# WilliamFlinchbaugh/Deep-RL-Battlespace

Hardware: AMD Instinct MI355X
Metric: agent-steps/sec (higher is better)
Workload: dtype f64/i16

## Files before the change

deep-rl-battlespace_amd/build.py:

```python
import os
import subprocess
import sys

HERE = os.path.dirname(os.path.abspath(__file__))
CSRC = os.path.join(HERE, "csrc")
INCLUDE = os.path.join(os.path.dirname(HERE), "include")
LIB = os.path.join(CSRC, "libbattlespace_hip.so")
COMMON = ["-O3", "--offload-arch=gfx950", "-fPIC", "-std=c++17", "-Wall", "-Wno-unused-function"]
STEP_FLAGS = ["-ffp-contract=off", "-mllvm", "-disable-machine-licm", "-mllvm", "-amdgpu-mfma-vgpr-form", "-mllvm", "-amdgpu-kernarg-preload-count=15"]
PER_CALL_FLAGS = STEP_FLAGS + ["-mllvm", "-amdgpu-sched-strategy=max-ilp"]
SOURCES = [(os.path.join(CSRC, "bsx_kernels.hip"), STEP_FLAGS),
           (os.path.join(CSRC, "bsx_step_per_call.hip"), PER_CALL_FLAGS),
           (os.path.join(CSRC, "bsx_step_multi_tick.hip"), STEP_FLAGS),
           (os.path.join(CSRC, "bsx_step_two_wave.hip"), PER_CALL_FLAGS),
           (os.path.join(CSRC, "bsx_step_rollout.hip"), STEP_FLAGS),
           (os.path.join(CSRC, "bsx_actor.hip"), ["-ffp-contract=off", "-mllvm", "-amdgpu-mfma-vgpr-form"]),
           (os.path.join(CSRC, "bsx_actor_grad.hip"), ["-ffp-contract=off", "-mllvm", "-amdgpu-mfma-vgpr-form"]),
           (os.path.join(CSRC, "bsx_replay.hip"), []),
           (os.path.join(CSRC, "bsx_advantage.hip"), ["-ffp-contract=off"]),
           (os.path.join(CSRC, "bsx_ppo_head.hip"), []),
           (os.path.join(CSRC, "bsx_adam_step.hip"), []),
           (os.path.join(CSRC, "bsx_ddpg_head.hip"), []),
           (os.path.join(CSRC, "bsx_shuffle.hip"), [])]


def _stale():
    if not os.path.exists(LIB):
        return True
    t = os.path.getmtime(LIB)
    import glob
    deps = [src for src, _ in SOURCES] + glob.glob(os.path.join(CSRC, "*.h")) + glob.glob(os.path.join(CSRC, "*.inl")) + \
        [os.path.join(INCLUDE, "battlespace_hip.h"), os.path.abspath(__file__)]
    return any(os.path.getmtime(d) > t for d in deps)


def build(force=False, verbose=False):
    if not force and not _stale():
        return LIB
    hipcc = os.environ.get("HIPCC", "/opt/rocm/bin/hipcc")
    from concurrent.futures import ThreadPoolExecutor

    def compile_one(item):
        src, extra = item
        obj = os.path.splitext(src)[0] + ".o"
        cmd = [hipcc, *COMMON, *extra, "-I", INCLUDE, "-c", src, "-o", obj]
        if verbose:
            print(" ".join(cmd), flush=True)
        subprocess.run(cmd, check=True)
        return obj
    with ThreadPoolExecutor(max_workers=len(SOURCES)) as pool:
        objs = list(pool.map(compile_one, SOURCES))
    cmd = [hipcc, "--offload-arch=gfx950", "-shared", "-fPIC", *objs, "-o", LIB]
    if verbose:
        print(" ".join(cmd), flush=True)
    subprocess.run(cmd, check=True)
    return LIB


if __name__ == "__main__":
    print(build(force="--force" in sys.argv, verbose=True))
```

deep-rl-battlespace_amd/csrc/bsx_kernels.hip:

```cpp

#include <array>
#include <mutex>
#include <unordered_map>

#include "bsx_config.h"
#include "bsx_args.h"
#include "bsx_state.h"
#include "bsx_rng.h"
#include "bsx_geometry.h"
#include "bsx_instinct.h"
#include "bsx_step_kernel.h"
#define BSX_INST_PER_CALL
#define BSX_INST_MULTI_TICK
#define BSX_INST_ROLLOUT
#include "bsx_step_split.h"
#define BSX_INST_SPLIT_MANY
#define BSX_INST_SPLIT
#define BSX_INST_SPLIT_CONT
#ifdef BSX_VARIANT
#define BSX_INST_KW
#else
#define BSX_INST_KW extern
#endif
#include "bsx_step_instances.h"
// ... 58 lines not shown
    if (!p.observe_only) {
        const int lane = tid & 63;
        const int64_t wb = int64_t(blockIdx.x) * (TPB / 64) + (tid >> 6);
        const unsigned long long resetting = __ballot(doit);
        if (resetting != 0ull && wb < wave_blocks(p.E, n)) {
            uint2* const pool = p.st.bent + size_t(wb) * POOL_CAP;
            const int pc = int(p.st.bcnt[wb]);
            int wpos = 0;
            for (int base = 0; base < pc; base += 64) {
                const int w = base + lane;
                const uint2 en = pool[w < pc ? w : 0];
                const bool stay = w < pc && ((resetting >> (en.x >> ENT_OWNER_SHIFT)) & 1ull) == 0ull;
                const unsigned long long kb = __ballot(stay);
                const int ps = wpos + __popcll(kb & ((1ull << lane) - 1ull));
                if (stay) pool[ps] = en;
                wpos += __popcll(kb);
            }
            if (lane == 0) p.st.bcnt[wb] = uint32_t(wpos);
        }
    }
    s_x[tid] = x; s_y[tid] = y; s_hp[tid] = valid ? hp : 0;
    __syncthreads();
    if (valid && p.obs) {
        const int team = a < n ? 0 : 1;
        write_obs<0>(p.obs + g * size_t(3 * n + 2), n, hp > 0, x, y, dir, a,
                     team == 0 ? er.bbx : er.brx, team == 0 ? er.bby : er.bry, gl, s_x, s_y, s_hp);
    }
}

__global__ void bsx_mark_done_kernel(uint2* envd, int64_t E) {
    const int64_t e = int64_t(blockIdx.x) * blockDim.x + threadIdx.x;
    if (e < E) envd[e] = make_uint2(1u << 27, 0u);
}

struct ExportArgs { StatePtrs st; int64_t E; int n; BsxExport out; int tie_tick; };

__global__ __launch_bounds__(TPB) void bsx_export_kernel(const ExportArgs p) {
    const int A = 2 * p.n;
    const size_t EA = size_t(p.E) * A;
    const size_t g = size_t(blockIdx.x) * TPB + threadIdx.x;
    if (g >= EA) return;
    const int64_t e = int64_t(g / A);
    const int a = int(g % A);
    const uint2 pw = p.st.plane[g];
    int x, y, hp;
    double dir;
    unpack_plane(pw, x, y, hp, dir);
    if (pw.y & PLANE_FRAC) dir = p.st.pdirf[g];
    const BsxExport& o = p.out;
    if (o.px) o.px[g] = x;
    if (o.py) o.py[g] = y;
    if (o.pdir) o.pdir[g] = dir;
    if (o.php) o.php[g] = hp;
    if (o.palive) o.palive[g] = hp > 0;
    const uint2 dw = p.st.envd[e];
    const EnvU ev = unpack_env(p.st.envc[e], dw.x);
    const int ptick = ev.tick - ((ev.done && ev.winner == BSX_WINNER_TIE && ev.tick >= p.tie_tick) ? 1 : 0);
    for (int k = 0; k < K; ++k) {
        const size_t i = g * K + k;
        if (o.bl_live) o.bl_live[i] = 0;
        if (o.bl_x) o.bl_x[i] = 0;
        if (o.bl_y) o.bl_y[i] = 0;
        if (o.bl_dir) o.bl_dir[i] = 0.0;
    }
    const int G = group_width(p.n), EPB = 64 / G;
    const int64_t wb = e / EPB;
    const uint32_t me = uint32_t(int(e % EPB) * G + a);
    const uint2* const pool = p.st.bent + size_t(wb) * POOL_CAP;
    const int cnt = int(p.st.bcnt[wb]);
    for (int j2 = 0; j2 < cnt; ++j2) {
        const uint32_t w = pool[j2].x;
        const int age = bullet_age(w);
        if ((w >> ENT_OWNER_SHIFT) != me || age == int(TOMBSTONE_AGE)) continue;
        int slot = (ptick - age + 1) % K;
        if (slot < 0) slot += K;
        const size_t i = g * K + slot;
        if (o.bl_live) o.bl_live[i] = 1;
        if (o.bl_x) o.bl_x[i] = bullet_x(w);
        if (o.bl_y) o.bl_y[i] = bullet_y(w);
        if (o.bl_dir) o.bl_dir[i] = p.st.bdir[size_t(slot) * EA + g];
    }
    if (a == 0) {
        if (o.base_xy) { o.base_xy[4 * e] = ev.brx; o.base_xy[4 * e + 1] = ev.bry; o.base_xy[4 * e + 2] = ev.bbx; o.base_xy[4 * e + 3] = ev.bby; }
        if (o.bhp) { o.bhp[2 * e] = ev.bhp_r; o.bhp[2 * e + 1] = ev.bhp_b; }
        if (o.tick) o.tick[e] = ev.tick;
        if (o.env_done) o.env_done[e] = ev.done;
        if (o.winner) o.winner[e] = ev.winner;
        if (o.counters) {
            const int* c4 = p.st.cnt + 4 * e;
            o.counters[4 * e] = c4[0]; o.counters[4 * e + 1] = c4[1]; o.counters[4 * e + 2] = c4[2]; o.counters[4 * e + 3] = c4[3];
        }
    }
}

struct InstinctArgs {
    const float* obs; void* actions; const double* rnd; int64_t E; int n; int team; int out_kind; int continuous;
    uint64_t seed; uint64_t seq; const uint64_t* seq_base; int64_t env_offset;
};

__global__ __launch_bounds__(TPB) void bsx_instinct_kernel(const InstinctArgs p) {
    const int A = 2 * p.n, D = 3 * p.n + 2;
    const size_t g = size_t(blockIdx.x) * TPB + threadIdx.x;
    if (g >= size_t(p.E) * A) return;
    const int a = int(g % A);
    const int tm = a < p.n ? 0 : 1;
    if (p.team != 2 && p.team != tm) return;
    const float* o = p.obs + g * D;
    double td, ta;
    const int act = instinct_choose([&](int k) { return o[k]; }, p.n, td, ta);
    if (!p.continuous) {
        if (p.out_kind == BSX_ACT_I32) static_cast<int32_t*>(p.actions)[g] = act;
        else static_cast<float4*>(p.actions)[g] = one_hot_scores(act);
        return;
    }
    double r0, n0, n1, n2;
    if (p.rnd) { r0 = p.rnd[4 * g]; n0 = p.rnd[4 * g + 1]; n1 = p.rnd[4 * g + 2]; n2 = p.rnd[4 * g + 3]; }
    else instinct_continuous_draws(p.seed, p.seq + (p.seq_base ? *p.seq_base : 0ull), uint64_t(p.env_offset) * uint64_t(A) + g, r0, n0, n1, n2);
    double* out = static_cast<double*>(p.actions) + 3 * g;
    instinct_continuous_action(td, ta, r0, n0, n1, n2, out[0], out[1], out[2]);
}

std::mutex g_family_mu;
std::unordered_map<const void*, int> g_family;
inline void family_forget(const void* state) {
    std::lock_guard<std::mutex> lk(g_family_mu);
    g_family.erase(state);
}
inline bool family_claim(const void* state, bool cont) {
    std::lock_guard<std::mutex> lk(g_family_mu);
    int& f = g_family[state];
    if (f == 0) f = cont ? 2 : 1;
    return f == (cont ? 2 : 1);
}
inline int grid_for(int64_t E, int n) {
    const int epb = TPB / group_width(n);
    return int((E + epb - 1) / epb);
}

inline bool narrow_offsets_ok(int64_t E, int n, uint32_t flags) {
    return !(flags & BSX_F_WIDE_OFFSETS) && uint64_t(E) * uint64_t(2 * n) * 200ull <= 0xFFFFFFFFull;
}
constexpr int64_t SPLIT_MAX_GAMES = 114688, SPLIT_MANY_MAX_GAMES = 65536, SPLIT_CONT_MAX_GAMES = 81920;
constexpr int64_t SPLIT_DRAW_MAX_GAMES = 98304;
constexpr int64_t SPLIT_MANY_FORM2_FROM = 32768;
template <bool CONT, bool MULTI>
inline bool split_applies(int n, const StepArgs& a, int64_t bound) {
    if (n != 1 || (a.flags & BSX_F_ONE_WAVE)) return false;
    if (CONT) return !MULTI && bound <= SPLIT_CONT_MAX_GAMES;
    return bound <= (MULTI ? SPLIT_MANY_MAX_GAMES : SPLIT_MAX_GAMES);
}

using StepKernel = void (*)(BSX_STEP_KERNEL_PARAMS);

template <class F>
StepKernel by_team_and_offsets(int n, bool off32, F f) {
    const auto w = [&](auto N) { return off32 ? f(N, std::true_type{}) : f(N, std::false_type{}); };
    switch (n) {
        case 1: return w(std::integral_constant<int, 1>{});
        case 2: return w(std::integral_constant<int, 2>{});
        case 3: return w(std::integral_constant<int, 3>{});
        case 4: return w(std::integral_constant<int, 4>{});
        default: return w(std::integral_constant<int, 0>{});
    }
}

template <bool CONT, bool MULTI, bool ACTOR, bool LG>
int launch_for_n(const StepArgs& a, int64_t bound, void* stream) {
    const int n = a.n;
    const bool two_wave = !ACTOR && split_applies<CONT, MULTI>(n, a, bound);
    const StepKernel k = by_team_and_offsets(n, narrow_offsets_ok(a.E, n, a.flags), [&](auto N_, auto OFF32_) -> StepKernel {
        constexpr int N = decltype(N_)::value;
        constexpr bool OFF32 = decltype(OFF32_)::value;
        if constexpr (ACTOR) {
            if constexpr (N == 0) return nullptr;
            else return bsx_step_kernel<N, CONT, true, true, false, OFF32>;
        } else {
            if constexpr (N == 1 && !(CONT && MULTI)) {
                if (two_wave) {
                    if constexpr (MULTI)
                        return bound > SPLIT_MANY_FORM2_FROM ? bsx_step_split_kernel<LG, OFF32, 2>
                                                             : bsx_step_split_kernel<LG, OFF32, 1>;
                    else if constexpr (CONT)
                        return bsx_step_split_kernel<false, OFF32, 0, true, true>;
                    else
                        return bound <= SPLIT_DRAW_MAX_GAMES ? bsx_step_split_kernel<LG, OFF32, 0, false, true>
                                                             : bsx_step_split_kernel<LG, OFF32, 0>;
                }
            }
            return bsx_step_kernel<N, CONT, MULTI, false, LG, OFF32>;
        }
    });
    const StepGeometry geo = step_geometry(ACTOR ? FORM_ROLLOUT : (two_wave ? FORM_TWO_WAVE : FORM_ONE_WAVE), bound, n);
    const dim3 grid(unsigned(geo.groups));
    const dim3 block(SPB * geo.waves);
    hipLaunchKernelGGL(k, grid, block, 0, static_cast<hipStream_t>(stream),
                       bound, a.st.envc, a.st.envd, a.st.plane, a.actions, a.st.bent, a.st.bcnt, a.action_kind, a);
    return int(hipGetLastError());
}

StepArgs step_args(void* state, int64_t E, int n, int T, float* rew, uint8_t* done, uint8_t* env_done, uint8_t* winner,
                   uint8_t* env_done_t, const BsxRewards* cfg, uint32_t flags, uint64_t seed, int64_t env_offset) {
    StepArgs a{};
    a.st = state_ptrs(state, E, n);
    a.E = E; a.n = n; a.T = T;
    a.rew = rew; a.done = done; a.env_done = env_done; a.winner = winner; a.env_done_t = env_done_t;
    a.cfg = *cfg; a.flags = flags; a.seed = seed; a.env_offset = env_offset; a.tie_tick = tie_tick_const(n);
    a.scripted_team = -1;
    return a;
}

struct StepCall { int64_t first = 0, count = -1; int T = 0; int store_all = 0; uint8_t* env_done_t = nullptr; };

template <bool CONT>
int step(const StepCall& c, void* state, int64_t E, int n, const void* actions, int action_kind, const double* u, float* obs, float* rew,
         uint8_t* done, uint8_t* env_done, uint8_t* winner, const BsxRewards* cfg, uint32_t flags, uint64_t seed, int64_t env_offset,
         void* stream) {
    const int T = c.T;
    const int64_t first = c.first, count = c.count < 0 ? E - first : c.count;
    if (T < 0 || T > BSX_MAX_T || first < 0 || count <= 0 || first > E - count || (first & 255) || ((first || count != E) && T != 0))
        return BSX_E_ARG;
    if (!obs || !rew || !done || !cfg || (!actions && (T || !(flags & BSX_F_EMPTY_CALL)))) return BSX_E_ARG;
    if (const int rc = check_games(state, E, n)) return rc;
    if (!aligned(obs, 4) || !aligned(rew, 4) || (u && !aligned(u, 8))) return BSX_E_ALIGN;
    if (!CONT && action_kind == BSX_ACT_LOGITS_F32 && !aligned(actions, 16)) return BSX_E_ALIGN;
    if (!CONT && action_kind != BSX_ACT_I32 && action_kind != BSX_ACT_LOGITS_F32) return BSX_E_ARG;
    if (CONT && action_kind != BSX_ACT_F32 && action_kind != BSX_ACT_F64 && action_kind != BSX_ACT_F32X4) return BSX_E_ARG;
    if (CONT && action_kind == BSX_ACT_F32X4 && !aligned(actions, 16)) return BSX_E_ALIGN;
    if (!family_claim(state, CONT)) return BSX_E_FAMILY;
    StepArgs a = step_args(state, E, n, T, rew, done, env_done, winner, c.env_done_t, cfg, flags, seed, env_offset);
    a.actions = actions; a.action_kind = action_kind; a.u = u; a.obs = obs;
    if (!actions) { a.actions = state; a.action_kind = -1; }
    const int64_t EA = E * 2 * n;
    a.act_tb = EA * (CONT ? (action_kind == BSX_ACT_F32 ? 12 : (action_kind == BSX_ACT_F64 ? 24 : 16)) : (action_kind == BSX_ACT_I32 ? 4 : 16));
    a.u_ts = EA;
    a.obs_ts = c.store_all ? EA * (3 * n + 2) : 0; a.rew_ts = c.store_all ? EA : 0; a.done_ts = c.store_all ? EA : 0;
    if (first) {
        const int64_t fa = first * 2 * n;
        const int64_t fb = first / (64 / group_width(n));
        a.st.envc += first; a.st.envd += first; a.st.cnt += 4 * first; a.st.plane += fa; a.st.pdirf += fa;
        a.st.bcnt += fb; a.st.bent += fb * POOL_CAP; a.st.bdir += fa; a.st.bd += fa;
        if (actions) a.actions = static_cast<const char*>(actions) + fa * (a.act_tb / EA);
        if (u) a.u += fa;
        a.obs += fa * (3 * n + 2); a.rew += fa; a.done += fa;
        if (env_done) a.env_done += first;
        if (winner) a.winner += first;
        a.env_offset += first;
    }
    const bool lg = !CONT && action_kind == BSX_ACT_LOGITS_F32;
    if (T == 0) return lg ? launch_for_n<CONT, false, false, !CONT>(a, count, stream) : launch_for_n<CONT, false, false, false>(a, count, stream);
    return lg ? launch_for_n<CONT, true, false, !CONT>(a, count, stream) : launch_for_n<CONT, true, false, false>(a, count, stream);
}

template <bool CONT>
int rollout(void* state, int64_t E, int n, int T, const float* weights, int precision, int scripted_team, uint64_t scripted_seed, float* obs,
            float* scores, float* rew, uint8_t* done, uint8_t* env_done, uint8_t* winner, uint8_t* env_done_t, const BsxRewards* cfg,
            uint32_t flags, const BsxActorNoise* noise, uint64_t actor_seed, uint64_t seq, const uint64_t* seq_base, uint64_t seed,
            int64_t env_offset, void* stream, bool gauss = false, const BsxGaussianHead* head = nullptr) {
    if (T < 1 || T > BSX_MAX_T || !weights || !obs || !scores || !rew || !done || !cfg || (flags & BSX_F_EMPTY_CALL) ||
        (precision != BSX_ACTOR_F32 && precision != BSX_ACTOR_BF16X3 && precision != BSX_ACTOR_BF16X6) || scripted_team < -1 || scripted_team > 1)
        return BSX_E_ARG;
    if (gauss && (!head || !head->log_std)) return BSX_E_ARG;
    if (const int rc = check_games(state, E, n, 256, ROLLOUT_MAX_N)) return rc;
    if (!aligned(weights, 16) || !aligned(scores, 16) || !aligned(obs, 4) || !aligned(rew, 4)) return BSX_E_ALIGN;
    BsxActorNoise nz = {};
    if (noise) nz = *noise;
    if (gauss) {
        if (nz.gaussian_std > 0.f || nz.ou_scale > 0.f || nz.sample_mode != 0 || nz.u_inject || nz.logp) return BSX_E_ARG;
        if (!aligned(head->log_std, 4) || (head->logp && !aligned(head->logp, 4))) return BSX_E_ALIGN;
    }
    if (nz.ou_scale > 0.f && (!nz.ou_state || !aligned(nz.ou_state, 16))) return nz.ou_state ? BSX_E_ALIGN : BSX_E_ARG;
    if (nz.z_inject || nz.u_inject) return BSX_E_ARG;
    if (nz.sample_mode != 0 && (nz.sample_mode != 1 || !(nz.temperature > 0.f) || CONT)) return BSX_E_ARG;
    if ((nz.logp && !aligned(nz.logp, 4)) || (nz.value_weights && !aligned(nz.value_weights, 16))) return BSX_E_ALIGN;
    if (nz.value_weights && (n != 1 || !nz.value || !aligned(nz.value, 4))) return BSX_E_ARG;
    if (!family_claim(state, CONT)) return BSX_E_FAMILY;
    const int64_t EA = E * 2 * n, D = 3 * n + 2;
    StepArgs a = step_args(state, E, n, T, rew, done, env_done, winner, env_done_t, cfg, flags, seed, env_offset);
    a.action_kind = CONT ? BSX_ACT_F32X4 : BSX_ACT_LOGITS_F32;
    a.obs = obs + EA * D; a.obs_ts = EA * D; a.rew_ts = EA; a.done_ts = EA;
    a.aw = weights; a.aprec = precision; a.scripted_team = scripted_team; a.obs0 = obs; a.scores = scores; a.scores_ts = EA * 4; a.nz = nz;
    a.aseed = actor_seed; a.aseq = seq; a.aseq_base = seq_base; a.iseed = scripted_seed;
    if (gauss) a.gh = *head;
    return launch_for_n<CONT, true, true, false>(a, E, stream);
}

const std::array<double2, 361>& heading_table() {
    static const std::array<double2, 361> lut = [] {
        std::array<double2, 361> t;
        const double st = 215 * 0.1;
        for (int d = 0; d <= 360; ++d) {
            const double ang = -(double(d) * DEG2RAD);
            t[d].x = st * cos(ang);
            t[d].y = st * sin(ang);
        }
        return t;
    }();
    return lut;
}

}

extern "C" {

int bsx_abi_version(void) { return BSX_ABI_VERSION; }

int bsx_build_flags(void) { return BUILD_FLAGS; }

int bsx_stream_synchronize(void* stream) { return int(hipStreamSynchronize(static_cast<hipStream_t>(stream))); }

int bsx_host_device_pointer(void* host, void** device) {
    if (!host || !device) return BSX_E_ARG;
    return int(hipHostGetDevicePointer(device, host, 0));
}

int bsx_tie_tick(int n) { return tie_tick_const(n); }

int bsx_state_bytes(int64_t E, int n, size_t* bytes) {
    if (const int rc = check_games(bytes, E, n, 1)) return rc;
    *bytes = make_layout(E, n).total;
    return 0;
}

int bsx_state_init(void* state, int64_t E, int n, void* stream) {
    if (const int rc = check_games(state, E, n)) return rc;
    const Layout L = make_layout(E, n);
    family_forget(state);
    hipStream_t s = static_cast<hipStream_t>(stream);
    hipError_t err = hipMemsetAsync(state, 0, L.total, s);
    if (err != hipSuccess) return int(err);
    const std::array<double2, 361>& lut = heading_table();
    err = hipMemcpyAsync(static_cast<char*>(state) + L.lut, lut.data(), sizeof(double2) * lut.size(), hipMemcpyHostToDevice, s);
    if (err != hipSuccess) return int(err);
    hipLaunchKernelGGL(bsx_mark_done_kernel, dim3(unsigned((E + TPB - 1) / TPB)), dim3(TPB), 0, s,
                       reinterpret_cast<uint2*>(static_cast<char*>(state) + L.envd), E);
    return int(hipGetLastError());
}

int bsx_state_release(void* state) {
    if (!state) return BSX_E_ARG;
    family_forget(state);
    return 0;
}

int bsx_reset(void* state, int64_t E, int n, const uint8_t* reset_mask, const int32_t* spawn, uint64_t seed,
              uint64_t nonce, int64_t env_offset, float* obs, void* stream) {
    if (const int rc = check_games(state, E, n)) return rc;
    if ((spawn && !aligned(spawn, 4)) || (obs && !aligned(obs, 4))) return BSX_E_ALIGN;
    if (!reset_mask) family_forget(state);
    ResetArgs a{state_ptrs(state, E, n), E, n, reset_mask, spawn, seed, nonce, env_offset, obs, 0};
// ... 142 lines not shown
```

deep-rl-battlespace_amd/csrc/bsx_state.h:

```cpp
#pragma once

namespace bsxk {


constexpr int K = BSX_BULLET_SLOTS;
constexpr int TPB = 256;
constexpr int SPB = 64;
constexpr int WPB = 1;

typedef float v4f_t __attribute__((ext_vector_type(4)));
template <class T> __device__ inline void out_store(T* p, T v) { __builtin_nontemporal_store(v, p); }

#define BSX_LDS(T, arr) ((__attribute__((address_space(3))) T*)(uintptr_t)(arr))

typedef uint32_t v4u_t __attribute__((ext_vector_type(4)));
template <bool NT, class T> __device__ inline void st_store(T* p, T v) {
    if (NT) __builtin_nontemporal_store(v, p);
    else *p = v;
}
__device__ inline v4u_t as_v4u(uint4 v) { return v4u_t{v.x, v.y, v.z, v.w}; }

constexpr int FIELD_W = 1200, FIELD_H = 800;
constexpr int PLANE_HW = 25, PLANE_HH = 24;
constexpr int PLANE_HP = 4;
constexpr double DEG2RAD = 3.141592653589793238462643383279502884 / 180.0;
constexpr double RAD2DEG = 180.0 / 3.141592653589793238462643383279502884;
constexpr double TWO_PI = 2.0 * 3.141592653589793;
constexpr double FIELD_DIAG = 1442.2205101855957;
constexpr double BULLET_STEP = 45.0;
constexpr double TIME_STEP = 0.1;

constexpr int POOL_CAP = 64 * BSX_BULLET_SLOTS;
struct Layout { size_t lut, envc, envd, cnt, plane, pdirf, bcnt, bent, bdir, bd, total; };

__host__ __device__ inline size_t align256(size_t v) { return (v + 255) & ~size_t(255); }
__host__ __device__ constexpr int group_width(int n) {
    int g = 2;
    while (g < 2 * n) g <<= 1;
    return g;
}
constexpr int ROLLOUT_MAX_N = 4;

enum StepForm : int { FORM_ONE_WAVE = 0, FORM_TWO_WAVE = 1, FORM_ROLLOUT = 2 };
struct StepGeometry { int64_t groups; int waves, pools; };
__host__ __device__ inline StepGeometry step_geometry(int form, int64_t games, int n) {
    const int G = group_width(n), epb = 64 / G;
    if (form == FORM_ROLLOUT) return {(games + 31) / 32, G / 2, G / 2};
    if (form == FORM_TWO_WAVE) return {(games + epb - 1) / epb, 2, 1};
    return {(games + WPB * epb - 1) / (WPB * epb), WPB, WPB};
}
__host__ __device__ inline int64_t wave_blocks(int64_t E, int n) {
    const StepGeometry w = step_geometry(n <= ROLLOUT_MAX_N ? FORM_ROLLOUT : FORM_ONE_WAVE, E, n);
    return w.groups * w.pools;
}

__host__ __device__ inline Layout make_layout(int64_t E, int n) {
    Layout L;
    const size_t EA = size_t(E) * size_t(2 * n);
    const size_t NB = size_t(wave_blocks(E, n));
    size_t o = 0;
    L.lut = o;   o = align256(o + 361 * sizeof(double2));
    L.envc = o;  o = align256(o + size_t(E) * sizeof(uint2));
    L.envd = o;  o = align256(o + size_t(E) * sizeof(uint2));
    L.cnt = o;   o = align256(o + size_t(E) * sizeof(int4));
    L.plane = o; o = align256(o + EA * sizeof(uint2));
    L.pdirf = o; o = align256(o + EA * sizeof(double));
    L.bcnt = o;  o = align256(o + NB * sizeof(uint32_t));
    L.bent = o;  o = align256(o + NB * size_t(POOL_CAP) * sizeof(uint2));
    L.bdir = o;  o = align256(o + size_t(K) * EA * sizeof(double));
    L.bd = o;    o = align256(o + size_t(K) * EA * sizeof(double2));
    L.total = o;
    return L;
}

struct StatePtrs {
    const double2* lut; uint2* envc; uint2* envd; int* cnt; uint2* plane; double* pdirf; uint32_t* bcnt; uint2* bent; double* bdir; double2* bd;
};
inline StatePtrs state_ptrs(void* base, int64_t E, int n) {
    Layout L = make_layout(E, n);
    char* b = static_cast<char*>(base);
    return StatePtrs{reinterpret_cast<const double2*>(b + L.lut), reinterpret_cast<uint2*>(b + L.envc), reinterpret_cast<uint2*>(b + L.envd),
                     reinterpret_cast<int*>(b + L.cnt), reinterpret_cast<uint2*>(b + L.plane), reinterpret_cast<double*>(b + L.pdirf),
                     reinterpret_cast<uint32_t*>(b + L.bcnt), reinterpret_cast<uint2*>(b + L.bent), reinterpret_cast<double*>(b + L.bdir),
                     reinterpret_cast<double2*>(b + L.bd)};
}

__device__ inline unsigned long long ballot64(bool p) { return __builtin_amdgcn_ballot_w64(p); }
__device__ inline bool any64(bool p) { return __builtin_amdgcn_ballot_w64(p) != 0ull; }
__device__ inline int lane_xor1(int v) { return __builtin_amdgcn_update_dpp(0, v, 0xB1, 0xF, 0xF, true); }
__device__ inline uint32_t rotl12(uint32_t v, int s) {
    return ((v << s) | (v >> (12 - s))) & 0xFFFu;
}
__device__ inline int sx16(uint32_t w) { return int(int16_t(w & 0xFFFFu)); }
__device__ inline int sy16(uint32_t w) { return int(int16_t(w >> 16)); }
__device__ inline uint32_t pack_xy(int x, int y) { return (uint32_t(x) & 0xFFFFu) | (uint32_t(y) << 16); }
constexpr uint32_t TOMBSTONE_AGE = 15;
constexpr uint32_t ENT_XY = 0x03FF07FFu, ENT_AGE = 0x7800u, ENT_EXACT = 0x8000u;
constexpr int ENT_OWNER_SHIFT = 26;
__device__ inline uint32_t pack_bullet(int x, int y, int age) { return uint32_t(x) | (uint32_t(age) << 11) | (uint32_t(y) << 16); }
__device__ inline int bullet_x(uint32_t w) { return int(w & 0x7FFu); }
__device__ inline int bullet_y(uint32_t w) { return int((w >> 16) & 0x3FFu); }
__device__ inline int bullet_age(uint32_t w) { return int((w >> 11) & 0xFu); }
typedef short s16x2 __attribute__((ext_vector_type(2)));
typedef uint32_t u32x2 __attribute__((ext_vector_type(2)));
__device__ inline s16x2 as_pk(uint32_t v) { return __builtin_bit_cast(s16x2, v); }
__device__ inline uint32_t pk_bits(s16x2 v) { return __builtin_bit_cast(uint32_t, v); }
constexpr uint32_t pk_const(int lo, int hi) { return (uint32_t(lo) & 0xFFFFu) | (uint32_t(hi) << 16); }
constexpr int PK_BIAS = 64;
__device__ inline int pk_any_negative(uint32_t t) { return int(t | (t << 16)) >> 31; }
constexpr float STEP_GUARD = 0x1p-17f;
__device__ inline uint32_t step_code(double dx, double dy, bool& exact) {
    const float dxf = float(dx), dyf = float(dy);
    const float fx = floorf(dxf), fy = floorf(dyf);
    const float rx = dxf - fx, ry = dyf - fy;
    exact = !(fminf(rx, ry) >= STEP_GUARD && fmaxf(rx, ry) <= 1.0f - STEP_GUARD);
    return pk_bits(__builtin_amdgcn_cvt_pk_i16(int(fx), int(fy)));
}
__device__ inline uint32_t step_pk(uint32_t xy, uint32_t code) {
    const s16x2 b = as_pk(xy) + as_pk(code);
    return pk_bits(b - (b >> 15));
}
__device__ inline int ring_pos(int ks, int back) { const int q = ks - back; return q + ((q >> 31) & BSX_BULLET_SLOTS); }

constexpr uint32_t PLANE_FRAC = 1u << 12;
__device__ inline void unpack_plane(const uint2 w, int& x, int& y, int& hp, double& dir) {
    x = sx16(w.x); y = sy16(w.x); hp = int((w.y >> 9) & 7u);
    dir = double(int(w.y & 511u));
}
__device__ inline uint2 pack_plane(int x, int y, int hp, double dir, bool frac) {
    return make_uint2(pack_xy(x, y), (uint32_t(int(dir)) & 511u) | (uint32_t(hp) << 9) | (frac ? PLANE_FRAC : 0u));
}
struct EnvU {
    int brx, bry, bbx, bby, bhp_r, bhp_b, tick, done, winner;
};
__device__ inline EnvU unpack_env(const uint2 c, const uint32_t d) {
    EnvU e;
    e.brx = sx16(c.x); e.bry = sy16(c.x); e.bbx = sx16(c.y); e.bby = sy16(c.y);
    e.bhp_r = int(d << 23) >> 23; e.bhp_b = int(d << 14) >> 23; e.tick = int((d >> 18) & 511u); e.done = int((d >> 27) & 1u); e.winner = int((d >> 28) & 3u);
    return e;
}
__device__ inline uint2 pack_envc(const EnvU& e) { return make_uint2(pack_xy(e.brx, e.bry), pack_xy(e.bbx, e.bby)); }
__device__ inline uint32_t pack_envd(const EnvU& e) {
    return (uint32_t(e.bhp_r) & 511u) | ((uint32_t(e.bhp_b) & 511u) << 9) | (uint32_t(e.tick) << 18) | (uint32_t(e.done) << 27) | (uint32_t(e.winner) << 28);
}
static_assert(5 * BSX_MAX_N < 256 && 12 * BSX_MAX_N < 256, "base hit points (start 5n, at most 12n hits in one call) fit 9 signed bits");

}
```

deep-rl-battlespace_amd/csrc/bsx_step_kernel.h:

```cpp
#pragma once

namespace bsxk {

__device__ inline int argmax4(float a, float b, float c, float d) {
    int am = 0;
    float best = a;
    const float v[3] = {b, c, d};
#pragma unroll
    for (int i = 0; i < 3; ++i)
        if (!(best != best) && (v[i] > best || v[i] != v[i])) { am = i + 1; best = v[i]; }
    return am;
}

struct StepArgs {
    StatePtrs st;
    int64_t E; int n;
    const void* actions; int action_kind;
    const double* u;
    float* obs; float* rew; uint8_t* done; uint8_t* env_done; uint8_t* winner;
    uint8_t* env_done_t;
    BsxRewards cfg;
    uint32_t flags; uint64_t seed; int64_t env_offset; int tie_tick;
    int T; int64_t act_tb , u_ts, obs_ts, rew_ts, done_ts ;
    const float* aw; int aprec; int scripted_team ; const float* obs0; float* scores; int64_t scores_ts; BsxActorNoise nz; uint64_t aseed, aseq; const uint64_t* aseq_base;
    uint64_t iseed;
    BsxGaussianHead gh;
};

#define BSX_STEP_KERNEL_PARAMS                                                                                                           \
    const int64_t E_, const uint2* const envc_, const uint2* const envd_, const uint2* const plane_, const void* const act_,               \
        const uint2* const bent_, const uint32_t* const bcnt_, const int kind_, const bsxk::StepArgs p_

template <int N>
__device__ inline void write_obs(float* __restrict__ out, int n, bool alive, int x, int y, double dir, int a,
                                 int ebx, int eby, int gl, const volatile int* s_x, const volatile int* s_y,
                                 const volatile int* s_hp) {
    const int D = 3 * n + 2;
    if (!alive || (DIAG & 1u)) {
        for (int i = 0; i < D; ++i) out[i] = -1.0f;
        return;
    }
    out[0] = obs_dist(x, y, ebx, eby);
    out[1] = obs_angle(x, y, dir, ebx, eby);
    const int eb = gl + (a < n ? n : 0);
    for (int j = 0; j < n; ++j) {
        if (s_hp[eb + j] > 0) {
            const int qx = s_x[eb + j], qy = s_y[eb + j];
            out[2 + 3 * j] = 1.0f;
            out[3 + 3 * j] = obs_dist(x, y, qx, qy);
            out[4 + 3 * j] = obs_angle(x, y, dir, qx, qy);
        } else {
            out[2 + 3 * j] = -1.0f; out[3 + 3 * j] = -1.0f; out[4 + 3 * j] = -1.0f;
        }
    }
}

enum Mode : int { M_INERT = 0, M_TIE = 1, M_PHYS = 2, M_RESET = 3 };

constexpr int tie_tick_const(int n) {
    const double max_time = double(10 + n * 2);
    double t = 0.0;
    int k = 0;
    do { t += 0.1; ++k; } while (!(t >= max_time));
    return k;
}
static_assert(tie_tick_const(1) == 121 && tie_tick_const(2) == 141 && tie_tick_const(3) == 161 && tie_tick_const(4) == 181 &&
              tie_tick_const(5) == 200, "time-limit tick");
static_assert(tie_tick_const(BSX_MAX_N) < 512, "the game clock fits the 9 bits of the game record");

template <class T> __device__ inline T* elem(T* base, uint32_t i) {
    typedef typename std::conditional<std::is_const<T>::value, const char, char>::type byte_t;
    return reinterpret_cast<T*>(reinterpret_cast<byte_t*>(base) + uint32_t(i * uint32_t(sizeof(T))));
}
template <class T> __device__ inline T* elem(T* base, size_t i) { return base + i; }
__device__ inline void end_of_tick() {
    __builtin_amdgcn_fence(__ATOMIC_RELEASE, "wavefront");
    __builtin_amdgcn_wave_barrier();
    __builtin_amdgcn_fence(__ATOMIC_ACQUIRE, "wavefront");
}
template <int N, bool CONT, bool MULTI, bool ACTOR = false, bool LG = false, bool OFF32 = false>
__global__ __launch_bounds__(SPB * (ACTOR ? group_width(N > 0 ? N : 1) / 2 : WPB)) __attribute__((amdgpu_waves_per_eu((ACTOR && N > 1) ? 2 : ((!ACTOR && MULTI && N == 2) ? 4 : 1))))
void bsx_step_kernel(BSX_STEP_KERNEL_PARAMS) {
    const StepArgs& p = p_;
    const unsigned stamp_row = blockIdx.x; (void)stamp_row;
    STAMP(8);
    typedef typename std::conditional<OFF32, uint32_t, size_t>::type ix_t;
    typedef typename std::conditional<OFF32, int32_t, int64_t>::type ixs_t;
    constexpr bool NT_STATE = !MULTI && N >= 2;
    constexpr int WAVES = ACTOR ? group_width(N > 0 ? N : 1) / 2 : WPB;
    const int n = (N > 0) ? N : p.n;
    const int A = 2 * n;
    const int G = group_width(n);
    const int EPB = SPB / G;
    const int wave = (WAVES > 1) ? int(threadIdx.x >> 6) : 0;
    const int tid = (WAVES > 1) ? int(threadIdx.x & 63) : int(threadIdx.x);
    const ixs_t wblk = (WAVES > 1) ? ixs_t(blockIdx.x) * WAVES + wave : ixs_t(blockIdx.x);
    const int a = tid & (G - 1);
    const ixs_t e = wblk * EPB + (tid / G);
    const bool env_ok = e < ixs_t(E_);
    const bool valid = env_ok && a < A;
    const ix_t EA = ix_t((MULTI || ACTOR) ? E_ : p.E) * ix_t(A);
    const ixs_t ec = env_ok ? e : ixs_t(E_ - 1);
    const ix_t g = ix_t(ec) * A + (a < A ? a : A - 1);
    constexpr int MANY = -1; constexpr bool DRAW = false;
#include "bsx_step_lds.inl"

    const bool has_act = kind_ >= 0;
    struct RawIn { int ai; float4 lg; float f0, f1, f2; double c0, c1, c2, uu; };
    auto load_inputs = [&](int t, RawIn& r) {
        const void* const at = MULTI ? static_cast<const void*>(static_cast<const char*>(act_) + int64_t(t) * p.act_tb) : act_;
        const double* const ut = (MULTI && p.u) ? p.u + int64_t(t) * p.u_ts : p.u;
        if (!CONT) {
            const char* const abase = static_cast<const char*>(at);
            if constexpr (LG) r.lg = *reinterpret_cast<const float4*>(elem(abase, has_act ? g * 16 : ix_t(0)));
            else r.ai = *reinterpret_cast<const int32_t*>(elem(abase, has_act ? g * 4 : ix_t(0)));
        } else if (has_act) {
            if (kind_ == BSX_ACT_F32) {
                const float* ap = static_cast<const float*>(at) + 3 * g;
                r.f0 = ap[0]; r.f1 = ap[1]; r.f2 = ap[2];
            } else if (kind_ == BSX_ACT_F32X4) {
                const float4 v = static_cast<const float4*>(at)[g];
                r.f0 = v.x; r.f1 = v.y; r.f2 = v.z;
            } else {
                const double* ap = static_cast<const double*>(at) + 3 * g;
                r.c0 = ap[0]; r.c1 = ap[1]; r.c2 = ap[2];
            }
        }
        __builtin_amdgcn_sched_barrier(0);
        if (ut) r.uu = ut[g];
    };
    int x = 0, y = 0, hp = 0;
    uint32_t games = 0;
    double dir = 0.0;
    EnvU er = {};
    const ix_t pool0 = ix_t(wblk) * ix_t(POOL_CAP);
    uint32_t pc = 0;
    uint2 pool_first = make_uint2(0u, 0u);
    RawIn rin = {}, rin_next = {};
    struct DecIn { int act; double a0, a1, a2, uu; };
    auto decode = [&](const RawIn& r) {
        DecIn d = {-1, 0.0, 0.0, 0.0, 0.0};
        if (has_act) {
            if (!CONT) {
                if constexpr (!LG) d.act = r.ai;
                else d.act = argmax4(r.lg.x, r.lg.y, r.lg.z, r.lg.w);
            } else if (kind_ == BSX_ACT_F32 || kind_ == BSX_ACT_F32X4) {
                d.a0 = double(r.f0); d.a1 = double(r.f1); d.a2 = double(r.f2);
            } else {
                d.a0 = r.c0; d.a1 = r.c1; d.a2 = r.c2;
            }
        }
        if (p.u) d.uu = r.uu;
        return d;
    };
    DecIn din_next = {-1, 0.0, 0.0, 0.0, 0.0};
    if (MULTI && !ACTOR) { load_inputs(0, rin_next); din_next = decode(rin_next); }
    if constexpr (ACTOR) {
        constexpr int D = 3 * N + 2;
        for (int i = int(threadIdx.x); i < 2 * N * bsx_actor::SMALL / 4; i += SPB * WAVES) {
            const int ag = i / (bsx_actor::SMALL / 4), j = i - ag * (bsx_actor::SMALL / 4);
            reinterpret_cast<float4*>(s_small)[i] =
                reinterpret_cast<const float4*>(p.aw + size_t(ag) * bsx_actor::blob_floats(D) + bsx_actor::off_small(D))[j];
        }
        if constexpr (N == 1) {
            if (p.nz.value_weights)
                for (int i = int(threadIdx.x); i < 2 * bsx_actor::SMALL / 4; i += SPB * WAVES) {
                    const int ag = i / (bsx_actor::SMALL / 4), j = i - ag * (bsx_actor::SMALL / 4);
                    reinterpret_cast<float4*>(s_small + 2 * bsx_actor::SMALL)[i] =
                        reinterpret_cast<const float4*>(p.nz.value_weights + size_t(ag) * bsx_actor::blob_floats(D) + bsx_actor::off_small(D))[j];
                }
        }
        const int64_t e_first = wblk * EPB;
        const int64_t nfl = min(int64_t(SPB), (E_ - e_first) * A) * D;
        if (G == A) {
            for (int i = tid; i < SPB * D; i += SPB) s_obs[i] = i < nfl ? p.obs0[size_t(e_first) * A * D + i] : -1.0f;
        } else {
            for (int k = 0; k < D; ++k) s_obs[tid * D + k] = valid ? p.obs0[g * D + k] : -1.0f;
        }
        __builtin_amdgcn_fence(__ATOMIC_RELEASE, "workgroup");
        if (WAVES > 1) __syncthreads(); else __builtin_amdgcn_wave_barrier();
        __builtin_amdgcn_fence(__ATOMIC_ACQUIRE, "workgroup");
    }

    for (int tk = 0; tk < (MULTI ? p.T : 1); ++tk) {
    ix_t gt = g, EAt = EA;
    uint64_t seed_t = p.seed;
    int64_t env_offset_t = p.env_offset;
    constexpr int TIE_C = tie_tick_const(N > 0 ? N : 1);
    int tie_tick = (N > 0) ? TIE_C : p.tie_tick;
    if (MULTI) {
        asm volatile("" : "+v"(gt));
        asm volatile("" : "+s"(EAt));
        asm volatile("" : "+s"(seed_t));
    }
    int tid_k = tid;
    if constexpr ((ACTOR && N > 1) || (MULTI && !ACTOR && N > 0 && ((OPAQUE_MULTI_MASK >> (((LG || CONT) ? 8 : 0) + N)) & 1))) asm volatile("" : "+v"(tid_k));
    typedef const StepArgs __attribute__((address_space(4))) StepArgsK;
    static_assert(alignof(StepArgs) == 8, "kernarg offset of StepArgs");
    const char __attribute__((address_space(4)))* ka = (const char __attribute__((address_space(4)))*)__builtin_amdgcn_kernarg_segment_ptr();
    if (MULTI) asm volatile("" : "+s"(ka));
    auto& p = [&]() -> decltype(auto) { if constexpr (MULTI) return (*reinterpret_cast<StepArgsK*>(ka + 64)); else return (p_); }();
    const int tid = tid_k, lane = tid, a = tid & (G - 1);
    const int gl = tid & ~(G - 1);
    const int team = (a < n) ? 0 : 1;
    const int eb = gl + (team == 0 ? n : 0);
    const double* const u_t = (MULTI && p.u) ? p.u + int64_t(tk) * p.u_ts : p.u;
    float* const obs_t = MULTI ? p.obs + int64_t(tk) * p.obs_ts : p.obs;
    float* const rew_t = MULTI ? p.rew + int64_t(tk) * p.rew_ts : p.rew;
    uint8_t* const done_t = MULTI ? p.done + int64_t(tk) * p.done_ts : p.done;
    STAMP(0);
    if (!MULTI || tk == 0) {
        const uint2 ecw = *elem(envc_, ix_t(ec));
        const uint2 edw = *elem(envd_, ix_t(ec));
        const uint2 prw = *elem(plane_, gt);
        double dirf = 0.0;
        pool_first = *elem(bent_, pool0 + ix_t(lane));
        if (!(DIAG & 2u)) pc = __builtin_amdgcn_readfirstlane(*elem(bcnt_, ix_t(wblk)));
        if constexpr (CONT) dirf = *elem(p.st.pdirf, gt);
        if (!MULTI) load_inputs(0, rin);
        if (!MULTI) {
            asm volatile("" : "+s"(seed_t), "+s"(env_offset_t));
            if (N == 0) asm volatile("" : "+s"(tie_tick));
        }
        unpack_plane(prw, x, y, hp, dir);
        if constexpr (CONT) dir = (prw.y & PLANE_FRAC) ? dirf : dir;
        er = unpack_env(ecw, edw.x);
        games = edw.y;
    } else {
        pool_first = *elem(bent_, pool0 + ix_t(lane));
    }
    const DecIn din = MULTI ? din_next : decode(rin);
    int act = din.act;
    double a0 = din.a0, a1 = din.a1, a2 = din.a2, uu_in = din.uu;
    constexpr bool R_BULLETS = true, R_MOVE = true, R_STAGE = true, R_GEOM = true, R_OUTCOME = true, R_ST_STATE = true, R_ST_OUT = true, R_POSE_LDS = false;
    constexpr int R_RDV_COUNTS = 0, R_GEOM_LDS = 0, R_PUB = 0, R_DRAW_LDS = 0;
    auto split_rendezvous = [] {};
#include "bsx_step_phase_actor.inl"
#include "bsx_step_phase_shot.inl"
#include "bsx_step_phase_move.inl"
#include "bsx_step_phase_geometry.inl"
#include "bsx_step_phase_bullets.inl"
#include "bsx_step_phase_outcome.inl"
#include "bsx_step_phase_stores.inl"
    STAMP(7);
    if (MULTI) {
        games += uint32_t(cnt_delta.x);
        end_of_tick();
        STAMP(9);
    }
    }
}

}
```

deep-rl-battlespace_amd/csrc/bsx_step_split.h:

```cpp
#pragma once

namespace bsxk {

template <bool LG, bool OFF32, int MANY = 0, bool CONT_ = false, bool DRAW = false>
__global__ __launch_bounds__(2 * SPB)
void bsx_step_split_kernel(BSX_STEP_KERNEL_PARAMS) {
    constexpr int N = 1;
    constexpr bool CONT = CONT_, MULTI = MANY != 0, ACTOR = false;
    static_assert(!CONT || (MANY == 0 && !LG), "continuous actions: the per-call form only");
    static_assert(!DRAW || MANY == 0, "the geometry wave's draw: the per-call form only");
    const StepArgs& p = p_;
    typedef typename std::conditional<OFF32, uint32_t, size_t>::type ix_t;
    typedef typename std::conditional<OFF32, int32_t, int64_t>::type ixs_t;
    constexpr bool NT_STATE = false;
    constexpr int WAVES = 1;
    const int n = 1, A = 2, G = 2, EPB = SPB / 2;
    const int wave = 0;
    const int role_wave = int(threadIdx.x >> 6);
    const unsigned stamp_row = blockIdx.x * 2u + unsigned(role_wave); (void)stamp_row;
    STAMP(8);
    STAMP_HWID();
    const int tid = int(threadIdx.x & 63);
    const ixs_t wblk = ixs_t(blockIdx.x);
    const int a = tid & (G - 1);
    const ixs_t e = wblk * EPB + (tid / G);
    const bool env_ok = e < ixs_t(E_);
    const bool valid = env_ok && a < A;
    const ix_t EA = ix_t(MULTI ? E_ : p.E) * ix_t(A);
    const ixs_t ec = env_ok ? e : ixs_t(E_ - 1);
    const ix_t g = ix_t(ec) * A + (a < A ? a : A - 1);
#include "bsx_step_lds.inl"
    auto split_rendezvous = [] {
        asm volatile("s_waitcnt lgkmcnt(0)\n\ts_barrier" ::: "memory");
    };
    const bool has_act = kind_ >= 0;
    struct RawIn { int ai; float4 lg; double uu; };
    struct DecIn { int act; double uu; };
    auto load_inputs = [&](int t, RawIn& r) {
        const char* const abase = static_cast<const char*>(act_) + (MULTI ? int64_t(t) * p.act_tb : int64_t(0));
        if constexpr (LG) r.lg = *reinterpret_cast<const float4*>(elem(abase, has_act ? g * 16 : ix_t(0)));
        else r.ai = *reinterpret_cast<const int32_t*>(elem(abase, has_act ? g * 4 : ix_t(0)));
        __builtin_amdgcn_sched_barrier(0);
        const double* const ut = (MULTI && p.u) ? p.u + int64_t(t) * p.u_ts : p.u;
        if (ut) r.uu = ut[g];
    };
    auto decode = [&](const RawIn& r) {
        DecIn d = {-1, 0.0};
        if (has_act) d.act = LG ? argmax4(r.lg.x, r.lg.y, r.lg.z, r.lg.w) : r.ai;
        if (p.u) d.uu = r.uu;
        return d;
    };
    const ix_t pool0 = ix_t(wblk) * ix_t(POOL_CAP);
    if constexpr (MANY != 0) {
        if (role_wave == 0) {
            __builtin_amdgcn_s_setprio(1);
            constexpr bool R_BULLETS = true, R_MOVE = true, R_STAGE = true, R_GEOM = false, R_OUTCOME = true, R_POSE_LDS = false;
            constexpr bool R_ST_STATE = MANY == 2, R_ST_OUT = false;
            constexpr int R_RDV_COUNTS = MANY == 2 ? 0 : 1, R_GEOM_LDS = 0, R_PUB = MANY == 2 ? 1 : 0, R_DRAW_LDS = 0;
            s_ov[tid] = 0ull;
#include "bsx_step_split_many_body.inl"
        } else if constexpr (MANY == 2) {
            constexpr bool R_BULLETS = false, R_GEOM = true, R_ST_STATE = false, R_ST_OUT = true;
            constexpr int R_GEOM_LDS = 0, R_PUB = 0;
#include "bsx_step_split_out_body.inl"
        } else {
            constexpr bool R_BULLETS = false, R_MOVE = true, R_STAGE = false, R_GEOM = true, R_OUTCOME = true, R_POSE_LDS = false;
            constexpr bool R_ST_STATE = true, R_ST_OUT = true;
            constexpr int R_RDV_COUNTS = 2, R_GEOM_LDS = 0, R_PUB = 0, R_DRAW_LDS = 0;
#include "bsx_step_split_many_body.inl"
        }
    } else {
        constexpr int R_PUB = 0;
        const int tk = 0;
        if (role_wave == 0) {
            __builtin_amdgcn_s_setprio(1);
            constexpr bool R_BULLETS = true, R_MOVE = true, R_STAGE = true, R_GEOM = false, R_OUTCOME = true, R_ST_STATE = true, R_ST_OUT = true;
            constexpr bool R_POSE_LDS = true;
            constexpr int R_RDV_COUNTS = 0, R_GEOM_LDS = 2, R_DRAW_LDS = DRAW ? 2 : 0;
            s_ov[tid] = 0ull;
#include "bsx_step_split_body.inl"
        } else {
#include "bsx_step_split_geom_body.inl"
        }
    }
}

}
```

Before: 23.98 billion.

## Pack game count, action kind and team size into one kernel argument

The game count, action kind and run-time team size are folded into a single 64-bit first kernel argument, so one fewer argument is needed and preloading can drop from 15 to 14 dwords. The StepArgs block offset moves to match, and the kernel reads n from the packed value instead of the argument struct. It also adds a compiler barrier on the DPP lane swap and a scheduling barrier before the continuous-action direction load to steer instruction scheduling. The risk is packing or offset mismatches, which static asserts are meant to catch.

```diff
diff --git a/deep-rl-battlespace_amd/build.py b/deep-rl-battlespace_amd/build.py
--- a/deep-rl-battlespace_amd/build.py
+++ b/deep-rl-battlespace_amd/build.py
@@ -7,7 +7,7 @@
 INCLUDE = os.path.join(os.path.dirname(HERE), "include")
 LIB = os.path.join(CSRC, "libbattlespace_hip.so")
 COMMON = ["-O3", "--offload-arch=gfx950", "-fPIC", "-std=c++17", "-Wall", "-Wno-unused-function"]
-STEP_FLAGS = ["-ffp-contract=off", "-mllvm", "-disable-machine-licm", "-mllvm", "-amdgpu-mfma-vgpr-form", "-mllvm", "-amdgpu-kernarg-preload-count=15"]
+STEP_FLAGS = ["-ffp-contract=off", "-mllvm", "-disable-machine-licm", "-mllvm", "-amdgpu-mfma-vgpr-form", "-mllvm", "-amdgpu-kernarg-preload-count=14"]
 PER_CALL_FLAGS = STEP_FLAGS + ["-mllvm", "-amdgpu-sched-strategy=max-ilp"]
 SOURCES = [(os.path.join(CSRC, "bsx_kernels.hip"), STEP_FLAGS),
            (os.path.join(CSRC, "bsx_step_per_call.hip"), PER_CALL_FLAGS),
diff --git a/deep-rl-battlespace_amd/csrc/bsx_kernels.hip b/deep-rl-battlespace_amd/csrc/bsx_kernels.hip
--- a/deep-rl-battlespace_amd/csrc/bsx_kernels.hip
+++ b/deep-rl-battlespace_amd/csrc/bsx_kernels.hip
@@ -234,6 +234,7 @@
 
 using StepKernel = void (*)(BSX_STEP_KERNEL_PARAMS);
 
+inline int runtime_team(int n) { return (n >= 1 && n <= 4) ? 0 : n; }
 template <class F>
 StepKernel by_team_and_offsets(int n, bool off32, F f) {
     const auto w = [&](auto N) { return off32 ? f(N, std::true_type{}) : f(N, std::false_type{}); };
@@ -276,7 +277,7 @@
     const dim3 grid(unsigned(geo.groups));
     const dim3 block(SPB * geo.waves);
     hipLaunchKernelGGL(k, grid, block, 0, static_cast<hipStream_t>(stream),
-                       bound, a.st.envc, a.st.envd, a.st.plane, a.actions, a.st.bent, a.st.bcnt, a.action_kind, a);
+                       step_pack_ek(bound, a.action_kind, runtime_team(n)), a.st.envc, a.st.envd, a.st.plane, a.actions, a.st.bent, a.st.bcnt, a);
     return int(hipGetLastError());
 }
 
diff --git a/deep-rl-battlespace_amd/csrc/bsx_state.h b/deep-rl-battlespace_amd/csrc/bsx_state.h
--- a/deep-rl-battlespace_amd/csrc/bsx_state.h
+++ b/deep-rl-battlespace_amd/csrc/bsx_state.h
@@ -34,11 +34,9 @@
 struct Layout { size_t lut, envc, envd, cnt, plane, pdirf, bcnt, bent, bdir, bd, total; };
 
 __host__ __device__ inline size_t align256(size_t v) { return (v + 255) & ~size_t(255); }
-__host__ __device__ constexpr int group_width(int n) {
-    int g = 2;
-    while (g < 2 * n) g <<= 1;
-    return g;
-}
+__host__ __device__ constexpr int group_width(int n) { return n <= 1 ? 2 : 1 << (32 - __builtin_clz(unsigned(2 * n - 1))); }
+static_assert(group_width(0) == 2 && group_width(1) == 2 && group_width(2) == 4 && group_width(3) == 8 && group_width(4) == 8 && group_width(5) == 16 &&
+              group_width(8) == 16 && group_width(9) == 32 && group_width(BSX_MAX_N) == 32, "group width");
 constexpr int ROLLOUT_MAX_N = 4;
 
 enum StepForm : int { FORM_ONE_WAVE = 0, FORM_TWO_WAVE = 1, FORM_ROLLOUT = 2 };
@@ -87,7 +85,11 @@
 
 __device__ inline unsigned long long ballot64(bool p) { return __builtin_amdgcn_ballot_w64(p); }
 __device__ inline bool any64(bool p) { return __builtin_amdgcn_ballot_w64(p) != 0ull; }
-__device__ inline int lane_xor1(int v) { return __builtin_amdgcn_update_dpp(0, v, 0xB1, 0xF, 0xF, true); }
+__device__ inline int lane_xor1(int v) {
+    int r = __builtin_amdgcn_update_dpp(0, v, 0xB1, 0xF, 0xF, true);
+    asm("" : "+v"(r));
+    return r;
+}
 __device__ inline uint32_t rotl12(uint32_t v, int s) {
     return ((v << s) | (v >> (12 - s))) & 0xFFFu;
 }
diff --git a/deep-rl-battlespace_amd/csrc/bsx_step_kernel.h b/deep-rl-battlespace_amd/csrc/bsx_step_kernel.h
--- a/deep-rl-battlespace_amd/csrc/bsx_step_kernel.h
+++ b/deep-rl-battlespace_amd/csrc/bsx_step_kernel.h
@@ -28,8 +28,30 @@
 };
 
 #define BSX_STEP_KERNEL_PARAMS                                                                                                           \
-    const int64_t E_, const uint2* const envc_, const uint2* const envd_, const uint2* const plane_, const void* const act_,               \
-        const uint2* const bent_, const uint32_t* const bcnt_, const int kind_, const bsxk::StepArgs p_
+    const int64_t ek_, const uint2* const envc_, const uint2* const envd_, const uint2* const plane_, const void* const act_,              \
+        const uint2* const bent_, const uint32_t* const bcnt_, const bsxk::StepArgs p_
+constexpr int STEP_PRELOAD_DWORDS = 14;
+constexpr int STEP_ARGS_OFFSET = 56;
+static_assert(STEP_ARGS_OFFSET == 4 * STEP_PRELOAD_DWORDS, "the argument block follows the preloaded arguments");
+constexpr int64_t step_pack_ek(int64_t games, int kind, int n_runtime) { return games | (int64_t(kind + 1 + (n_runtime << 8)) << 32); }
+constexpr int64_t step_games(int64_t ek) { return int64_t(uint32_t(ek)); }
+template <int N> constexpr int step_kind(int64_t ek) { return (N > 0 ? int(ek >> 32) : (int(ek >> 32) & 255)) - 1; }
+constexpr int step_n_runtime(int64_t ek) { return int(ek >> 40); }
+template <int N> constexpr bool step_ek_round_trips(int64_t games, int kind, int n) {
+    return step_games(step_pack_ek(games, kind, N > 0 ? 0 : n)) == games && step_kind<N>(step_pack_ek(games, kind, N > 0 ? 0 : n)) == kind &&
+           (N > 0 || step_n_runtime(step_pack_ek(games, kind, n)) == n);
+}
+constexpr bool step_ek_round_trips_all() {
+    for (int kind : {-1, BSX_ACT_I32, BSX_ACT_LOGITS_F32, BSX_ACT_F32, BSX_ACT_F64, BSX_ACT_F32X4})
+        for (int64_t games : {int64_t(1), int64_t(65536), int64_t(1) << 30})
+            if (!step_ek_round_trips<1>(games, kind, 1) || !step_ek_round_trips<4>(games, kind, 4) ||
+                !step_ek_round_trips<0>(games, kind, 5) || !step_ek_round_trips<0>(games, kind, BSX_MAX_N))
+                return false;
+    return true;
+}
+static_assert(step_ek_round_trips_all(), "game count, action kind and run-time team size share the first kernel argument");
+static_assert(BSX_MAX_N < (1 << 22), "the run-time team size fits beside the action kind");
+#define BSX_STEP_UNPACK_EK const int64_t E_ = bsxk::step_games(ek_); const int kind_ = bsxk::step_kind<N>(ek_);
 
 template <int N>
 __device__ inline void write_obs(float* __restrict__ out, int n, bool alive, int x, int y, double dir, int a,
@@ -82,13 +104,14 @@
 __global__ __launch_bounds__(SPB * (ACTOR ? group_width(N > 0 ? N : 1) / 2 : WPB)) __attribute__((amdgpu_waves_per_eu((ACTOR && N > 1) ? 2 : ((!ACTOR && MULTI && N == 2) ? 4 : 1))))
 void bsx_step_kernel(BSX_STEP_KERNEL_PARAMS) {
     const StepArgs& p = p_;
+    BSX_STEP_UNPACK_EK
     const unsigned stamp_row = blockIdx.x; (void)stamp_row;
     STAMP(8);
     typedef typename std::conditional<OFF32, uint32_t, size_t>::type ix_t;
     typedef typename std::conditional<OFF32, int32_t, int64_t>::type ixs_t;
     constexpr bool NT_STATE = !MULTI && N >= 2;
     constexpr int WAVES = ACTOR ? group_width(N > 0 ? N : 1) / 2 : WPB;
-    const int n = (N > 0) ? N : p.n;
+    const int n = (N > 0) ? N : step_n_runtime(ek_);
     const int A = 2 * n;
     const int G = group_width(n);
     const int EPB = SPB / G;
@@ -199,7 +222,7 @@
     static_assert(alignof(StepArgs) == 8, "kernarg offset of StepArgs");
     const char __attribute__((address_space(4)))* ka = (const char __attribute__((address_space(4)))*)__builtin_amdgcn_kernarg_segment_ptr();
     if (MULTI) asm volatile("" : "+s"(ka));
-    auto& p = [&]() -> decltype(auto) { if constexpr (MULTI) return (*reinterpret_cast<StepArgsK*>(ka + 64)); else return (p_); }();
+    auto& p = [&]() -> decltype(auto) { if constexpr (MULTI) return (*reinterpret_cast<StepArgsK*>(ka + STEP_ARGS_OFFSET)); else return (p_); }();
     const int tid = tid_k, lane = tid, a = tid & (G - 1);
     const int gl = tid & ~(G - 1);
     const int team = (a < n) ? 0 : 1;
@@ -216,7 +239,7 @@
         double dirf = 0.0;
         pool_first = *elem(bent_, pool0 + ix_t(lane));
         if (!(DIAG & 2u)) pc = __builtin_amdgcn_readfirstlane(*elem(bcnt_, ix_t(wblk)));
-        if constexpr (CONT) dirf = *elem(p.st.pdirf, gt);
+        if constexpr (CONT) { if (!MULTI) __builtin_amdgcn_sched_barrier(0); dirf = *elem(p.st.pdirf, gt); }
         if (!MULTI) load_inputs(0, rin);
         if (!MULTI) {
             asm volatile("" : "+s"(seed_t), "+s"(env_offset_t));
diff --git a/deep-rl-battlespace_amd/csrc/bsx_step_split.h b/deep-rl-battlespace_amd/csrc/bsx_step_split.h
--- a/deep-rl-battlespace_amd/csrc/bsx_step_split.h
+++ b/deep-rl-battlespace_amd/csrc/bsx_step_split.h
@@ -10,6 +10,7 @@
     static_assert(!CONT || (MANY == 0 && !LG), "continuous actions: the per-call form only");
     static_assert(!DRAW || MANY == 0, "the geometry wave's draw: the per-call form only");
     const StepArgs& p = p_;
+    BSX_STEP_UNPACK_EK
     typedef typename std::conditional<OFF32, uint32_t, size_t>::type ix_t;
     typedef typename std::conditional<OFF32, int32_t, int64_t>::type ixs_t;
     constexpr bool NT_STATE = false;
```

Result: no change. 24.19 billion, median of 6 (+0.8%).
